# emstoudenmire/TNML

Hardware: AMD Instinct MI355X
Metric: two-site bond updates/sec (higher is better)
Workload: dtype f64; 1 GPU; fixedL N=784, maxm=120, 60000 images (BASELINE config 3: its 60 000 images on 1 GPU instead of 8), Npass=4, lambda=0.001, minm=120, fp64 throughout; random-init W at m=maxm; timed bonds 405..202 (consecutive interior bonds, Label-carrying shiftE on each, m=119); global_images=60000, sites=784, maxm=120, parallelism=dp1 (image sharding + RCCL all-reduce), rccl_ranks=1

## Files before the change

### include/tnml.h

```cpp
#ifndef TNML_H
#define TNML_H

#include <stdint.h>

#ifdef __cplusplus
extern "C" {
#endif

#define TNML_NL 10
#define TNML_MAX_PASS 64

typedef struct tnml_ctx tnml_ctx;

enum { TNML_F32 = 0, TNML_F64_E32 = 1, TNML_F64 = 2, TNML_BF16 = 3, TNML_BF16X3 = 4 };
enum { TNML_SVD_SYEVD = 0, TNML_SVD_ROCSOLVER = 1, TNML_SVD_STEDC = 2 };
enum { TNML_MODE_FIXEDL = 0, TNML_MODE_SINGLE = 1 };

typedef struct {
    int device;
    int rank, nranks;
    int N;
    int NT_local;
    int64_t NT_total;
    int maxm;
// ... 96 lines not shown
    int bond, half;
    int64_t count;
    int64_t ncorrect;
    double cost;
    double label_cost[TNML_NL];
} tnml_heldout_report;
int tnml_heldout_attach(tnml_ctx* train, tnml_ctx* heldout);
int tnml_heldout_detach(tnml_ctx* train);
int tnml_heldout_read(tnml_ctx* train, tnml_heldout_report* rep);

int tnml_truncate(const double* p, int n, int maxm, int minm, double cutoff, double* truncerr);
void tnml_sweepnext(int* b, int* ha, int N);
void tnml_shard_bounds(int64_t NT_total, int nranks, int rank, int64_t* begin, int64_t* end);

int tnml_profile_enable(tnml_ctx* ctx, int on);
int tnml_profile_select(tnml_ctx* ctx, const char* class_name);
int tnml_profile_count(tnml_ctx* ctx);
int tnml_profile_get(tnml_ctx* ctx, int idx, char* name64, int64_t* launches, double* total_ms);
int tnml_profile_reset(tnml_ctx* ctx);
int tnml_synchronize(tnml_ctx* ctx);
int tnml_set_option(tnml_ctx* ctx, const char* name, int value);
int tnml_set_option_real(tnml_ctx* ctx, const char* name, double value);
int tnml_split_stats(tnml_ctx* ctx, int64_t* spec_splits, int64_t* roll_backs, double* roll_back_ms);
int tnml_svd_stats(tnml_ctx* ctx, int64_t* fallbacks, int64_t* cluster_repairs, double* dev_before_polish, double* dev_after_first_polish);
int64_t tnml_device_bytes(tnml_ctx* ctx);

int64_t tnml_estimate_bytes(const tnml_config* cfg);
int tnml_device_memory(int device, int64_t* free_bytes, int64_t* total_bytes);
int tnml_plan_maxm(const tnml_config* cfg, int wanted, int floor_m, int64_t budget_bytes);

#define TNML_LIN_MAX_COLS 16
typedef struct tnml_lin tnml_lin;
int tnml_lin_create(tnml_lin** out, int device, int N);
int tnml_lin_destroy(tnml_lin* ctx);
const char* tnml_lin_last_error(const tnml_lin* ctx);
int tnml_lin_set_data_u8(tnml_lin* ctx, int NT, const uint8_t* pixels, const int32_t* labels);
int tnml_lin_set_data_f64(tnml_lin* ctx, int NT, const double* features, const int32_t* labels);
int tnml_lin_set_labels(tnml_lin* ctx, int K, const int32_t* labels);
int tnml_lin_cg_start(tnml_lin* ctx, const double* V, double lambda);
int tnml_lin_cg_run(tnml_lin* ctx, int npass, double* costs);
int tnml_lin_get_v(tnml_lin* ctx, double* V);
int tnml_lin_evaluate(tnml_lin* ctx, const double* V, int64_t* ncorrect, double* cnl);

#ifdef __cplusplus
}
#endif
// ... 2 lines not shown
```

### tnml_amd/csrc/kernels_res.hip

```cpp
#include "tnml_internal.h"

typedef double f64x4r __attribute__((ext_vector_type(4)));

#define FR_TI 32
#define FR_ROWS(NKA) (4 * (NKA) + 4)
#define FR_EIS(NKA) (FR_ROWS(NKA) * FR_TI)
#define FR_LDS_DOUBLES_N(NKA) (2 * FR_EIS(NKA) + 2 * 64 * FR_TI + 2 * 4 * TNML_NL * FR_TI)
#define FR_LDS_DOUBLES FR_LDS_DOUBLES_N(30)

static __device__ __forceinline__ void fr_barrier() {
    asm volatile("s_waitcnt lgkmcnt(0)" ::: "memory");
    __builtin_amdgcn_s_barrier();
    asm volatile("" ::: "memory");
}

template <int PS, int PK, int ABL, int NKA = 30, bool GEN = false, int NST = 8>
__global__ __launch_bounds__(768) void k_fwd_res(FwdResArgs A) {
    static_assert(GEN || NKA == 30, "the constant-extent form is the 120 x 120 bond");
    static_assert(NST == 8 || (NST == 4 && GEN), "four or eight streaming steps per tile");
    constexpr int EIS = FR_EIS(NKA);
    const int mI = GEN ? A.mI : 120, mO = GEN ? A.mO : 120, Kp = GEN ? A.Kp : 240, Np = GEN ? A.Np : 240;
    extern __shared__ __attribute__((aligned(16))) double fr_lds[];
    double* EIs = fr_lds;
    double* Us = EIs + 2 * EIS;
// ... 184 lines not shown
        for (int it = 1; it <= niter; ++it) {
            const long long c0 = ABL == 5 ? clock64() : 0;
            const int tile = pair + (it - 1) * npairs;
            label_dot(tile, it < niter ? tile + npairs : tile, Us + ((it - 1) & 1) * 64 * FR_TI, red + (it & 1) * 4 * TNML_NL * FR_TI, [&]() {
                x_stage(it + 1 < niter ? pair + (it + 1) * npairs : tile, (it + 1) & 1);
                if (it >= 2) finalize(pair + (it - 2) * npairs, red + ((it - 1) & 1) * 4 * TNML_NL * FR_TI);
            });
            if constexpr (NST == 8) asm volatile("s_waitcnt vmcnt(40)" ::: "memory");
            else                    asm volatile("s_waitcnt vmcnt(20)" ::: "memory");
            const long long c1 = ABL == 5 ? clock64() : 0;
            fr_barrier();
            if (ABL == 5) { const long long c2 = clock64(); t_dot += c1 - c0; t_bar += c2 - c1; }
        }
        if (ABL == 5 && A.dbg && blockIdx.x < 16 && lane == 0) { long long* d = A.dbg + (blockIdx.x * 12 + wid) * 4; d[0] = t_dot; d[1] = 0; d[2] = t_bar; d[3] = niter; }
        asm volatile("s_waitcnt vmcnt(0)" ::: "memory");
        finalize(pair + (niter - 1) * npairs, red + (niter & 1) * 4 * TNML_NL * FR_TI);
        fr_barrier();
#undef FR_WAIT
    }
}

#define SR_TI 64

template <int NKS>
__global__ __launch_bounds__(512) void k_shift_res(ShiftResArgs A) {
    constexpr int ROWS = 4 * NKS + 2;
    constexpr int NP = 2 * NKS + 1;
    extern __shared__ __attribute__((aligned(16))) double sr_lds[];
    const int tid = threadIdx.x, lane = tid & 63, w = __builtin_amdgcn_readfirstlane(tid >> 6);
    const int NTp = A.NTp, tpl = NTp / SR_TI;
    const int G = gridDim.x;
    const int niter = (A.ntiles - (int)blockIdx.x + G - 1) / G;
    const unsigned lds0 = __builtin_amdgcn_readfirstlane((unsigned)(size_t)((__attribute__((address_space(3))) char*)sr_lds));
    const unsigned doff = (unsigned)(((size_t)(lane >> 5) * NTp + 2 * (lane & 31)) * sizeof(double));
    auto dma16 = [&](const double* base, unsigned voff, unsigned dst) {
        unsigned keep;
        asm volatile("s_mov_b32 %0, m0\n\ts_mov_b32 m0, %2\n\ts_nop 0\n\tglobal_load_lds_dwordx4 %1, %3\n\ts_mov_b32 m0, %0" : "=&s"(keep) : "v"(voff), "s"(dst), "s"(base) : "memory");
    };
    const unsigned doff0 = (unsigned)((2 * (lane & 31)) * sizeof(double));
    auto stage = [&](int t, int buf) {
        const int l = t / tpl, n0 = (t - l * tpl) * SR_TI;
        const double* eb = A.EI + (size_t)l * A.EI_lstride + n0;
#pragma unroll
        for (int r = 0; r < 8; ++r) {
            int p = w + 8 * r;
            if (p >= NP) p -= NP;
            if (p >= NP) p -= NP;
            const int r0 = 2 * p < A.mI ? 2 * p : 0;
            dma16(p == NP - 1 ? A.phiI + n0 : eb + (size_t)r0 * NTp, (p != NP - 1 && 2 * p == A.mI - 1) ? doff0 : doff, lds0 + (unsigned)((buf * ROWS * SR_TI + 2 * p * SR_TI) * sizeof(double)));
        }
    };
    const int CT = A.Np >> 4;
    const bool split = CT <= 4;
    const int ct = split ? (w & 3) : w;
    const bool act = ct < CT;
    const bool do0 = !split || w < 4, do1 = !split || w >= 4;
    double me[NKS], mo[NKS];
    {
        const int g = lane >> 4, i = lane & 15;
#pragma unroll
        for (int ks = 0; ks < NKS; ++ks) {
            const bool in = act && 2 * (4 * ks + g) + 1 < A.Kp;
            me[ks] = in ? A.M[(size_t)(2 * (4 * ks + g)) * A.Np + 16 * ct + i] : 0.;
            mo[ks] = in ? A.M[(size_t)(2 * (4 * ks + g) + 1) * A.Np + 16 * ct + i] : 0.;
        }
    }
    if (niter > 0) stage(blockIdx.x, 0);
    asm volatile("s_waitcnt vmcnt(0)" ::: "memory");
    fr_barrier();
    double ob[8];
    double* obp = nullptr;
    for (int it = 0; it < niter; ++it) {
        const int t = blockIdx.x + it * G;
        const int l = t / tpl, n0 = (t - l * tpl) * SR_TI;
        int ln = lane;
        asm volatile("" : "+v"(ln));
        int g = ln >> 4, i = ln & 15;
        if (obp) {
#pragma unroll
            for (int q = 0; q < 8; ++q) { const int y = 16 * ct + g + 4 * (q & 3); if (y < A.mO) obp[(size_t)(4 * (q & 3)) * NTp + 16 * (q >> 2)] = ob[q]; }
        }
        if (it + 1 < niter) stage(t + G, (it + 1) & 1);
        const double* Eb = sr_lds + (it & 1) * ROWS * SR_TI;
        double* op = A.out + (size_t)l * A.out_lstride + (size_t)(16 * ct + g) * NTp + n0 + i;
        if (act) {
#pragma unroll
            for (int pass = 0; pass < 2; ++pass) {
                if (pass == 0 ? !do0 : !do1) continue;
                const double* ep0 = Eb + g * SR_TI + 32 * pass + i;
                const double* ep1 = ep0 + 16;
                f64x4r ce0 = {0., 0., 0., 0.}, co0 = {0., 0., 0., 0.}, ce1 = {0., 0., 0., 0.}, co1 = {0., 0., 0., 0.};
                double a0 = ep0[0], b0 = ep1[0], a1 = ep0[4 * SR_TI], b1 = ep1[4 * SR_TI];
// ... 28 lines not shown
            if (do1) obp = op + 32;
        }
        asm volatile("s_waitcnt vmcnt(0)" ::: "memory");
        fr_barrier();
    }
    if (obp) {
        const int g = lane >> 4;
#pragma unroll
        for (int q = 0; q < 8; ++q) { const int y = 16 * ct + g + 4 * (q & 3); if (y < A.mO) obp[(size_t)(4 * (q & 3)) * NTp + 16 * (q >> 2)] = ob[q]; }
    }
}

static const int sr_nks_list[] = {12, 16, 18, 20, 22, 24, 26, 28, 30};
static int sr_nks_for(int mI) {
    for (int v : sr_nks_list) if (4 * v >= mI) return v;
    return 0;
}
bool shift_res_applies(int mI, int mO) { return mI >= 33 && sr_nks_for(mI) != 0 && mO >= 1 && mO <= 128; }

template <int NKS>
static int shift_res_go(tnml_ctx* c, const ShiftResArgs& a, int grid) {
    const size_t lds = sizeof(double) * 2 * (4 * NKS + 2) * SR_TI;
    if (!c->attr_sr[NKS]) {
        if (hipFuncSetAttribute(reinterpret_cast<const void*>(k_shift_res<NKS>), hipFuncAttributeMaxDynamicSharedMemorySize, (int)lds) != hipSuccess)
            return tnml_fail(c, "shift_res: cannot reserve %zu bytes of LDS", lds);
        c->attr_sr[NKS] = true;
    }
    ProfScope ps(c, KC_FGEMM_SHIFT);
    hipLaunchKernelGGL(k_shift_res<NKS>, dim3(grid), dim3(512), lds, c->stream, a);
    return 0;
}
int launch_shift_res(tnml_ctx* c, const ShiftResArgs& a_in) {
    ShiftResArgs a = a_in;
    if (a.NTp % SR_TI) return tnml_fail(c, "shift_res: image count not a multiple of %d", SR_TI);
    if (((size_t)a.L * a.EI_lstride) * sizeof(double) >= ((size_t)1 << 32)) return tnml_fail(c, "shift_res: environment larger than 4 GB (32-bit lane offsets)");
    if (!shift_res_applies(a.mI, a.mO) || a.Np % 16 || a.Np < a.mO || a.Np > 128) return tnml_fail(c, "shift_res: bond dimensions %d x %d (packed %d) not served", a.mI, a.mO, a.Np);
    if (!c->cu_count) { hipDeviceProp_t pr; c->cu_count = hipGetDeviceProperties(&pr, c->cfg.device) == hipSuccess ? pr.multiProcessorCount : 256; }
    a.ntiles = a.L * (a.NTp / SR_TI);
    int grid = c->cu_count;
    if (c->res_grid > 0 && c->res_grid < grid) grid = c->res_grid;
    if (grid > a.ntiles) grid = a.ntiles;
    switch (sr_nks_for(a.mI)) {
        case 12: TCK((shift_res_go<12>(c, a, grid))); break;
        case 16: TCK((shift_res_go<16>(c, a, grid))); break;
        case 18: TCK((shift_res_go<18>(c, a, grid))); break;
        case 20: TCK((shift_res_go<20>(c, a, grid))); break;
        case 22: TCK((shift_res_go<22>(c, a, grid))); break;
        case 24: TCK((shift_res_go<24>(c, a, grid))); break;
        case 26: TCK((shift_res_go<26>(c, a, grid))); break;
        case 28: TCK((shift_res_go<28>(c, a, grid))); break;
        default: TCK((shift_res_go<30>(c, a, grid))); break;
    }
    HIPCK(c, hipGetLastError());
    return 0;
}

static __device__ __forceinline__ void res_wave_partials(double val, int lab, int cor, bool pap, double* out, int lane) {
    if (pap) {
        const double s = wave_sum(val);
        if (lane < 12) out[lane] = lane == 11 ? s : 0.;
        return;
    }
    double mine = 0.;
#pragma unroll
    for (int t = 0; t < TNML_NL; ++t) {
        const double s = wave_sum(lab == t ? val : 0.);
        if (lane == t) mine = s;
    }
    const double sc = wave_sum((double)cor);
    if (lane == 10) mine = sc;
    if (lane < 12) out[lane] = mine;
}

__global__ __launch_bounds__(256) void k_pfinish(PfinishArgs A) {
    const int tid = threadIdx.x, lane = tid & 63;
    const int NTp = A.NTp;
    const int ni = blockIdx.x * 256 + tid;
    if (A.conv && A.conv[0] != 0.) return;
    const int lab = A.label[ni];
// ... 106 lines not shown
```

### tnml_amd/csrc/tnml_abi.hip

```cpp
#include <algorithm>
#include <climits>
#include <cmath>
#include <cstdarg>
#include <cstdlib>
#include <cstring>

#include "tnml_internal.h"

static std::string g_create_err;

int tnml_fail(tnml_ctx* c, const char* fmt, ...) {
    char buf[512];
    va_list ap; va_start(ap, fmt); vsnprintf(buf, sizeof buf, fmt, ap); va_end(ap);
    if (c) { c->err = buf; if (c->local && c->coll_depth > 0) local_comm_abort(c); } else g_create_err = buf;
    return 1;
}
const char* tnml_last_error(const tnml_ctx* c) { return c ? c->err.c_str() : g_create_err.c_str(); }
const char* tnml_last_warning(const tnml_ctx* c) { return c ? c->warn.c_str() : ""; }
struct CollScope { tnml_ctx* c; explicit CollScope(tnml_ctx* c_) : c(c_) { ++c->coll_depth; } ~CollScope() { --c->coll_depth; } };
static int ho_locked(tnml_ctx* c, const char* who, bool train_too = false) {
    if (c->held) return tnml_fail(c, "%s: the context is attached as a held-out set (tnml_heldout_detach first)", who);
    if (train_too && c->ho) return tnml_fail(c, "%s: a held-out context is attached to this context (tnml_heldout_detach first)", who);
    return 0;
}
// ... 46 lines not shown
}
int tnml_profile_reset(tnml_ctx* c) {
    prof_resolve(c);
    for (int i = 0; i < KC_COUNT; ++i) { c->prof_launches[i] = 0; c->prof_ms[i] = 0.; }
    return 0;
}
enum OptKind { OPT_BOOL, OPT_INT, OPT_REAL };
enum OptHook { HK_NONE, HK_REUSE_P, HK_DEFER_TAIL, HK_CHECK_REPLICAS, HK_ENV_BUDGET, HK_COMM_TIMEOUT, HK_FAIL_SPLIT, HK_SVD_PRINT, HK_CG_METHOD, HK_NOISE };
struct OptDef {
    const char* name; const char* env; OptKind kind;
    int tnml_ctx::* ifield; double tnml_ctx::* rfield;
    double lo, hi; OptHook hook;
};
static const OptDef k_options[] = {
    {"fast_cg",          "TNML_FAST_CG",        OPT_BOOL, &tnml_ctx::fast_cg,             nullptr,          0, 1,       HK_NONE},
    {"reuse_p",          "TNML_REUSE_P",        OPT_BOOL, &tnml_ctx::reuse_p,             nullptr,          0, 1,       HK_REUSE_P},
    {"fuse_z",           "TNML_FUSE_Z",         OPT_BOOL, &tnml_ctx::fuse_z,              nullptr,          0, 1,       HK_NONE},
    {"merged_cg",        "TNML_MERGED_CG",      OPT_INT,  &tnml_ctx::merged_cg,           nullptr,          0, 2,       HK_NONE},
    {"defer_tail",       "TNML_DEFER_TAIL",     OPT_BOOL, &tnml_ctx::defer_tail,          nullptr,          0, 1,       HK_DEFER_TAIL},
    {"check_replicas",   "TNML_CHECK_REPLICAS", OPT_INT,  &tnml_ctx::check_replicas_mode, nullptr,          0, 2,       HK_CHECK_REPLICAS},
    {"fused_fwd",        "TNML_FUSED_FWD",      OPT_INT,  &tnml_ctx::fused_fwd,           nullptr,          0, INT_MAX, HK_NONE},
    {"fwd_res",          "TNML_FWD_RES",        OPT_INT,  &tnml_ctx::fwd_res,             nullptr,          0, 3,       HK_NONE},
    {"shift_res",        "TNML_SHIFT_RES",      OPT_INT,  &tnml_ctx::shift_res,           nullptr,          0, 2,       HK_NONE},
    {"res_grid",         nullptr,               OPT_INT,  &tnml_ctx::res_grid,            nullptr,          0, INT_MAX, HK_NONE},
    {"res_pace",         "TNML_RES_PACE",       OPT_INT,  &tnml_ctx::res_pace,            nullptr,          0, 4,       HK_NONE},
    {"grad_quad",        "TNML_GRAD_QUAD",      OPT_INT,  &tnml_ctx::grad_quad,           nullptr,          0, 2,       HK_NONE},
    {"grad_pair",        "TNML_GRAD_PAIR",      OPT_BOOL, &tnml_ctx::grad_pair,           nullptr,          0, 1,       HK_NONE},
    {"bgemm_wgs",        "TNML_BGEMM_WGS",      OPT_INT,  &tnml_ctx::bgemm_wgs,           nullptr,          0, INT_MAX, HK_NONE},
    {"bgemm_per",        "TNML_BGEMM_PER",      OPT_INT,  &tnml_ctx::bgemm_per,           nullptr,          0, 1 << 20, HK_NONE},
    {"sytrd_exit",       nullptr,               OPT_BOOL, &tnml_ctx::sytrd_exit,          nullptr,          0, 1,       HK_NONE},
    {"bgs_chol",         "TNML_BGS_CHOL",       OPT_BOOL, &tnml_ctx::bgs_chol,            nullptr,          0, 1,       HK_NONE},
    {"spec_split",       "TNML_SPEC_SPLIT",     OPT_BOOL, &tnml_ctx::spec_split,          nullptr,          0, 1,       HK_NONE},
    {"debug_fail_split", nullptr,               OPT_INT,  &tnml_ctx::debug_fail_split,    nullptr,         -1, INT_MAX, HK_FAIL_SPLIT},
    {"bf16_grad",        nullptr,               OPT_BOOL, &tnml_ctx::bf16_grad,           nullptr,          0, 1,       HK_NONE},
    {"bf16_once",        nullptr,               OPT_BOOL, &tnml_ctx::bf16_once,           nullptr,          0, 1,       HK_NONE},
    {"env_async",        nullptr,               OPT_BOOL, &tnml_ctx::env_async,           nullptr,          0, 1,       HK_NONE},
    {"env_budget_mb",    nullptr,               OPT_INT,  nullptr,                        nullptr,          0, INT_MAX, HK_ENV_BUDGET},
    {"comm_timeout_s",   nullptr,               OPT_INT,  &tnml_ctx::comm_timeout_s,      nullptr,          1, INT_MAX, HK_COMM_TIMEOUT},
    {"cg_method",        nullptr,               OPT_INT,  &tnml_ctx::cg_method,           nullptr,          0, 2,       HK_CG_METHOD},
    {"debug_nudge_rank", nullptr,               OPT_INT,  &tnml_ctx::debug_nudge_rank,    nullptr,         -1, INT_MAX, HK_NONE},
    {"mc_spin_max",      nullptr,               OPT_INT,  &tnml_ctx::mc_spin_max,         nullptr,         -1, INT_MAX, HK_NONE},
    {"svd_print",        "TNML_SVD_PRINT",      OPT_INT,  &tnml_ctx::svd_print,           nullptr,         -2, INT_MAX, HK_SVD_PRINT},
    {"fg64_cfg",         "TNML_FG64_CFG",       OPT_INT,  &tnml_ctx::opt_fg64_cfg,        nullptr,          0, 2,       HK_NONE},
    {"ldot_cfg",         "TNML_LDOT_CFG",       OPT_INT,  &tnml_ctx::opt_ldot_cfg,        nullptr,          0, 2,       HK_NONE},
    {"pcut",             nullptr,               OPT_REAL, nullptr,                        &tnml_ctx::pcut,  0, HUGE_VAL, HK_NONE},
    {"noise",            nullptr,               OPT_REAL, nullptr,                        &tnml_ctx::noise, 0, HUGE_VAL, HK_NOISE},
// ... 93 lines not shown
    c->small_elems = m * NTp;
    c->big_elems = TNML_NL * m * NTp;
    c->svd_n = 2 * c->maxm;
    c->slab_bytes = (size_t)128 * Kmax * Kmax * 4 * (c->f64() ? 2 : 1);
    c->partial_cap = (int)(NTp / 64);
    c->sM_cap = std::max(40 * m * m, (size_t)TNML_NL * Kmax * ru16(c->maxm));
    c->ebt_cap = c->bf16() ? bf16e_env_elems(c->maxm, c->NTp, c->bf16() == 2) : 0;
    c->mbt_cap = c->bf16() ? bf16e_m_elems(c->maxm, c->bf16() == 2) : 0;
    c->W.resize(c->N + 2);
    c->env.resize(c->N + 2);
    c->spare_small.assign(4, nullptr);
    c->spare_big.assign(c->c0 > 0 ? 2 : 0, nullptr);
}
struct DevBuf { void** slot; size_t bytes; bool on, site; };
static std::vector<DevBuf> device_buffers(tnml_ctx* c) {
    const size_t NTp = c->NTp, m = c->maxm, n = c->svd_n, esz = c->esz(), eesz = c->eesz(), D = sizeof(double);
    std::vector<DevBuf> v;
    auto add = [&](auto& p, size_t bytes, bool on = true) { v.push_back({(void**)&p, bytes, on, false}); };
    add(c->phi, c->N * 2 * NTp * eesz); add(c->label, NTp * sizeof(int)); add(c->ones, NTp * eesz);
    add(c->U, c->big_elems * esz); add(c->P, TNML_NL * NTp * esz); add(c->dP, TNML_NL * NTp * esz); add(c->Pp, TNML_NL * NTp * esz);
    add(c->Zp, c->small_elems * esz); add(c->Mf, c->mcap * sizeof(float)); add(c->slab, c->slab_bytes);
    add(c->partials, c->partial_cap * 12 * D); add(c->partials2, c->partial_cap * 12 * D); add(c->counters, 16 * sizeof(unsigned));
    add(c->Ppart, 2 * TNML_NL * NTp * D, c->cfg.dtype == TNML_F64 && c->cfg.mode == TNML_MODE_FIXEDL && m >= 33);
    add(c->ebt, c->ebt_cap * sizeof(unsigned short), c->bf16() != 0); add(c->mbt, c->mbt_cap * sizeof(unsigned short), c->bf16() != 0);
    add(c->vB, c->mcap * D); add(c->vR, c->mcap * D); add(c->vP, c->mcap * D); add(c->arbuf, (c->mcap + TNML_TAILN) * D); add(c->locals, 32 * D);
    add(c->scal, (SC_N + 4 * TNML_MAX_PASS) * D);
    add(c->vpart, (1024 + 16) * D);
    add(c->tB, c->mcap * D); add(c->tB2, c->mcap * D);
    add(c->sM, c->sM_cap * D); add(c->sG, n * n * D); add(c->sD, n * D); add(c->sE, 2 * n * D); add(c->sF, (n * m + 2 * TNML_NL * m * m) * D);
    add(c->sInfo, 4 * sizeof(int)); add(c->fprint, 2 * sizeof(unsigned long long));
    add(c->sE2, n * D); add(c->sTau, n * D); add(c->sV, n * n * D); add(c->sC, n * n * D);
    add(c->sW, (n + 8) * D);
    add(c->sScr, std::max<size_t>(5 * n * m, TEIG_SCRATCH_DOUBLES) * D); add(c->sS, m * m * D); add(c->sCm, m * m * D); add(c->sQ1, n * m * D); add(c->sDev, 4 * D);
    add(c->mc_xbuf, eigh_mc_xbuf_bytes(), n > 240);
    for (int j = 1; j <= c->N; ++j) v.push_back({(void**)&c->W[j].a, 2 * m * m * (j == c->c0 ? TNML_NL : 1) * D, true, true});
    for (auto& p : c->spare_small) v.push_back({(void**)&p, 2 * m * m * D, true, true});
    for (auto& p : c->spare_big) v.push_back({(void**)&p, 2 * m * m * TNML_NL * D, true, true});
    return v;
}
static int dalloc(tnml_ctx* c, void** p, size_t bytes) {
    hipError_t e = hipMalloc(p, bytes);
    if (e != hipSuccess) return tnml_fail(c, "hipMalloc of %zu bytes failed: %s", bytes, hipGetErrorString(e));
    c->bytes += (int64_t)bytes;
    return 0;
}
int ctx_alloc_doubles(tnml_ctx* c, double** p, size_t n) { return dalloc(c, (void**)p, (n ? n : 1) * sizeof(double)); }
// ... 211 lines not shown
    else if (ncclCommCount(c->comm, &cnt) != ncclSuccess) return tnml_fail(c, "ncclCommCount failed");
    if (nranks_in_comm) *nranks_in_comm = cnt;
    if (cnt != c->cfg.nranks) return tnml_fail(c, "communicator has %d ranks, context was created for %d", cnt, c->cfg.nranks);
    TCK(check_W(c));
    if (c->pend_count) return tnml_fail(c, "tnml_replica_check: a bond update is in flight");
    TCK(replica_fingerprint(c, 1, c->N, c->tail + TNML_FPSLOT));
    TCK(allreduce(c, c->tail + TNML_FPSLOT, 8));
    double h[8];
    HIPCK(c, hipMemcpyAsync(h, c->tail + TNML_FPSLOT, sizeof h, hipMemcpyDeviceToHost, c->stream));
    SYNCK(c, c->stream);
    if (!fingerprint_agrees(h, c->cfg.nranks)) return tnml_fail(c, "replicas of the weight MPS differ between ranks");
    return 0;
}

static int set_labels(tnml_ctx* c, const int32_t* labels) {
    std::vector<int> lab(c->NTp, -1);
    for (int i = 0; i < c->NT; ++i) {
        if (labels[i] < 0 || labels[i] >= TNML_NL) return tnml_fail(c, "label %d of image %d out of range", labels[i], i);
        lab[i] = labels[i];
    }
    HIPCK(c, hipMemcpy(c->label, lab.data(), sizeof(int) * c->NTp, hipMemcpyHostToDevice));
    return 0;
}
int tnml_set_data_u8(tnml_ctx* c, const uint8_t* pixels, const int32_t* labels) {
    TCK(ho_locked(c, "tnml_set_data_u8", true));
    HIPCK(c, hipSetDevice(c->cfg.device));
    TCK(set_labels(c, labels));
    uint8_t* d_pix = nullptr;
    const size_t nb = (size_t)c->NT * c->N;
    HIPCK(c, hipMalloc((void**)&d_pix, nb));
    HIPCK(c, hipMemcpy(d_pix, pixels, nb, hipMemcpyHostToDevice));
    int rc = launch_features_u8(c, d_pix, c->N, c->NT, c->NTp, c->phi);
    (void)hipStreamSynchronize(c->stream);
    (void)hipFree(d_pix);
    if (rc) return rc;
    c->data_set = true; c->currb = -1; c->p_valid = false; c->sweep_start = false;
    return 0;
}
int tnml_set_data_phi(tnml_ctx* c, const double* phi, const int32_t* labels) {
    TCK(ho_locked(c, "tnml_set_data_phi", true));
    HIPCK(c, hipSetDevice(c->cfg.device));
    TCK(set_labels(c, labels));
    const size_t ne = (size_t)c->N * 2 * c->NTp;
    if (c->env64()) {
        std::vector<double> h(ne, 0.);
        for (int i = 0; i < c->NT; ++i) for (int j = 0; j < c->N; ++j) for (int s = 0; s < 2; ++s)
            h[((size_t)j * 2 + s) * c->NTp + i] = phi[((size_t)i * c->N + j) * 2 + s];
        HIPCK(c, hipMemcpy(c->phi, h.data(), sizeof(double) * ne, hipMemcpyHostToDevice));
    } else {
        std::vector<float> h(ne, 0.f);
        for (int i = 0; i < c->NT; ++i) for (int j = 0; j < c->N; ++j) for (int s = 0; s < 2; ++s)
            h[((size_t)j * 2 + s) * c->NTp + i] = (float)phi[((size_t)i * c->N + j) * 2 + s];
        HIPCK(c, hipMemcpy(c->phi, h.data(), sizeof(float) * ne, hipMemcpyHostToDevice));
    }
    c->data_set = true; c->currb = -1; c->p_valid = false; c->sweep_start = false;
    return 0;
}

int tnml_set_site(tnml_ctx* c, int j, int ml, int mr, int has_label, const double* A) {
    TCK(ho_locked(c, "tnml_set_site", true));
    if (j < 1 || j > c->N) return tnml_fail(c, "tnml_set_site: site %d out of range", j);
    if (c->single() && has_label) return tnml_fail(c, "tnml_set_site: the per-label variant has no Label index");
    if ((j == c->c0) != (has_label != 0)) return tnml_fail(c, "Label Index not on site %d", c->c0);
    if (ml < 1 || mr < 1 || ml > c->maxm || mr > c->maxm) return tnml_fail(c, "tnml_set_site: bond dimension outside 1..maxm");
    if ((j == 1 && ml != 1) || (j == c->N && mr != 1)) return tnml_fail(c, "tnml_set_site: edge sites must have outer dimension 1");
    SiteT& s = c->W[j];
    s.ml = ml; s.mr = mr; s.L = has_label ? TNML_NL : 1; s.set = true;
    HIPCK(c, hipMemcpy(s.a, A, sizeof(double) * (size_t)ml * 2 * mr * s.L, hipMemcpyHostToDevice));
    c->currb = -1; c->p_valid = false; c->sweep_start = false;
    return 0;
}
// ... 181 lines not shown
    if (Lout_p) *Lout_p = Lout;
    c->env_epoch += 1;
    PackDesc d;
    d.TO = 1; d.L = A.L; d.st = 0; d.ss = A.ml; d.sl = (long)2 * A.ml * A.mr;
    if (from_left) { d.nx = A.ml; d.sx = 1; d.ny = A.mr; d.sy = 2 * A.ml; }
    else           { d.nx = A.mr; d.sx = 2 * A.ml; d.ny = A.ml; d.sy = 1; }
    d.Kp = ru16(2 * d.nx); d.Np = ru16(d.ny);
    if ((size_t)d.L * d.Kp * d.Np > c->sM_cap || (size_t)d.L * d.Kp * d.Np > c->mcap)
        return tnml_fail(c, "shift: packed site matrix of site %d (%d x %d x %d) exceeds the workspace", cs, d.L, d.Kp, d.Np);
    if (c->f64()) {
        TCK(launch_pack(c, d, A.a, c->sM, nullptr));
        Fgemm64Args f;
        f.EI = src ? src : c->ones;
        f.EI_lstride = (Le == TNML_NL) ? (size_t)m_in * c->NTp : 0;
        f.mI = m_in; f.phiI = phi_site(c, cs);
        f.M = c->sM; f.M_lstride = (A.L == TNML_NL) ? (size_t)d.Kp * d.Np : 0; f.Kp = d.Kp; f.Np = d.Np;
        f.phiO = nullptr;
        f.out = (double*)dst; f.out_lstride = (size_t)m_out * c->NTp; f.mO = m_out;
        f.NTp = c->NTp; f.L = Lout; f.env64 = c->env64(); f.out32 = !c->env64() && !acc_out;
        if (c->shift_res && c->env64() && !acc_out && src && Le == TNML_NL && A.L == 1 && shift_res_applies(m_in, m_out) && d.Np <= 128 &&
            (c->shift_res >= 2 || c->NTp >= 7680) &&
            (size_t)TNML_NL * m_in * c->NTp * sizeof(double) < ((size_t)1 << 32)) {
            ShiftResArgs sa{(const double*)src, (size_t)m_in * c->NTp, (const double*)phi_site(c, cs), c->sM, (double*)dst, (size_t)m_out * c->NTp, m_out, c->NTp, Lout, m_in, d.Kp, d.Np};
            return launch_shift_res(c, sa);
        }
        return launch_fgemm64(c, f);
    }
    TCK(launch_pack(c, d, A.a, nullptr, c->Mf));
    FgemmArgs f;
    f.EI = src ? (const float*)src : (const float*)c->ones;
    f.EI_lstride = (Le == TNML_NL) ? (size_t)m_in * c->NTp : 0;
    f.mI = m_in; f.phiI = (const float*)phi_site(c, cs);
    f.M = c->Mf; f.M_lstride = (A.L == TNML_NL) ? (size_t)d.Kp * d.Np : 0; f.Kp = d.Kp; f.Np = d.Np;
    f.phiO = nullptr;
    f.out = (float*)dst; f.out_lstride = (size_t)m_out * c->NTp; f.mO = m_out;
    f.NTp = c->NTp; f.L = Lout;
    return launch_fgemm(c, f);
}
static int shift_site(tnml_ctx* c, int cs, int ps, bool from_left) {
    const SiteT& A = c->W[cs];
    const bool has_prev = ps >= 1 && ps <= c->N;
    if (has_prev && !c->env[ps].built()) return tnml_fail(c, "shift: environment of site %d missing", ps);
    EnvProtect keep(c, has_prev ? ps : 0, cs, c->currb > 0 ? c->currb - 1 : 0, c->currb > 0 ? c->currb + 2 : 0);
    if (has_prev) TCK(env_ensure(c, ps));
    const int m_in = from_left ? A.ml : A.mr, m_out = from_left ? A.mr : A.ml;
    const int Le = has_prev ? c->env[ps].L : 1;
// ... 927 lines not shown
```

### tnml_amd/csrc/tnml_internal.h

```cpp
#pragma once
#include <hip/hip_runtime.h>
#include <rocblas/rocblas.h>
#include <rocsolver/rocsolver.h>
#include <rccl/rccl.h>

#include <cstdint>
#include <cstdio>
#include <string>
#include <utility>
#include <vector>

#include "../../include/tnml.h"

#define TNML_NTPAD 256

enum KClass {
    KC_FGEMM_FWD = 0, KC_FGEMM_SHIFT, KC_LABELDOT, KC_ZPRIME, KC_BGEMM, KC_SLABRED, KC_PACK, KC_VEC,
    KC_SMALLGEMM, KC_SVD, KC_ALLREDUCE, KC_PUPDATE, KC_FWD_FUSED, KC_FWD_RES, KC_GRAD_QUAD, KC_COUNT
};
static const char* const kclass_names[KC_COUNT] = {
    "fgemm_fwd", "fgemm_shift", "labeldot", "zprime", "bgemm", "slab_reduce", "pack", "cg_vec",
    "small_gemm", "svd", "allreduce", "p_update", "fwd_fused", "fwd_res", "grad_quad"};

struct EnvSlot {
// ... 135 lines not shown
    int merged_cg = 1;
    int defer_tail = 1;
    int carry_slot = -1;
    long allreduce_calls = 0, bcast_calls = 0;
    double* scal = nullptr;
    double* cgtrace = nullptr;
    double* vpart = nullptr;
    int cg_pass = 0;
    int rr_slot = 0;
    double* h_scal = nullptr;
    double *tB = nullptr, *tB2 = nullptr;
    size_t mcap = 0;
    size_t sM_cap = 0;
    double *sM = nullptr, *sG = nullptr, *sD = nullptr, *sE = nullptr, *sF = nullptr;
    double *sE2 = nullptr, *sTau = nullptr, *sV = nullptr, *sC = nullptr;
    double *sW = nullptr, *sScr = nullptr, *sS = nullptr, *sCm = nullptr, *sQ1 = nullptr, *sDev = nullptr;
    void* mc_xbuf = nullptr;
    unsigned mc_epoch = 0;
    int mc_spin_max = -1;
    bool attr_sr[32] = {false}, attr_fr[4][32] = {{false}};
    int res_pace = 0;
    int fwd_res = 1;
    int shift_res = 1;
    int res_grid = 0;
    int grad_quad = 1;
    bool attr_gq = false, attr_gp = false;
    int grad_pair = 1;
    int bgemm_per = 0;
    int bgemm_wgs = 0;
    unsigned* counters = nullptr;
    double* Ppart = nullptr;
    bool attr_sytrd = false, attr_invit = false, attr_fused = false;
    int cu_count = 0;
    int spec_split = 1; bool force_safe = false; long spec_redos = 0, spec_splits = 0;
    int debug_fail_split = -1;
    long spec_splits_total = 0; double redo_ms = 0.; std::vector<std::pair<hipEvent_t, hipEvent_t>> redo_events;
    std::vector<double*> spare_small, spare_big;
    double* hrep = nullptr;
    double* hmir = nullptr;
    double* hcost = nullptr;
    int last_dn_pairs = 0;
    size_t hrep_stride = 0;
    double svd_last_dev0 = 0., svd_last_dev1 = 0.;
    long svd_fallbacks = 0, svd_cholqr = 0;
    int svd_print = -2, svd_calls = 0, svd_dumped = 0;
    std::string svd_dump;
// ... 136 lines not shown
bool fwd_res_applies(int mI, int mO);
int launch_fwd_res(tnml_ctx* c, const FwdResArgs& a);
struct PfinishArgs {
    int npart;
    const double* Ppart;
    const double* P; const double* Pp; const double* alpha;
    const double* conv;
    const int* label; int NTp;
    double* Pout; double* dP;
    int mode;
    double* partials;
    unsigned* counter;
    double* out; int only_sum;
};
int launch_pfinish(tnml_ctx* c, const PfinishArgs& a);
struct ShiftResArgs {
    const double* EI; size_t EI_lstride;
    const double* phiI;
    const double* M;
    double* out; size_t out_lstride; int mO;
    int NTp, L;
    int mI, Kp, Np;
    int ntiles = 0;
};
bool shift_res_applies(int mI, int mO);
int launch_shift_res(tnml_ctx* c, const ShiftResArgs& a);

struct PackDesc {
    int nx, ny, TO, L;
    long sx, ss, sy, st, sl;
    int Kp, Np;
};
static inline rocblas_status dgemm_strips(rocblas_handle h, rocblas_operation ta, rocblas_operation tb, int M, int N, int K,
                                          const double* A, int lda, const double* B, int ldb, double* C, int ldc, int strips) {
    const double one = 1.0, zero = 0.0;
    if (strips <= 1 || N % strips || N / strips < 16) return rocblas_dgemm(h, ta, tb, M, N, K, &one, A, lda, B, ldb, &zero, C, ldc);
    const int ns = N / strips;
    const rocblas_stride sb = tb == rocblas_operation_none ? (rocblas_stride)ns * ldb : (rocblas_stride)ns;
    return rocblas_dgemm_strided_batched(h, ta, tb, M, ns, K, &one, A, lda, 0, B, ldb, sb, &zero, C, ldc, (rocblas_stride)ns * ldc, strips);
}
int launch_pack(tnml_ctx* c, const PackDesc& d, const double* T, double* Md, float* Mf, double* zero = nullptr, int nzero = 0);
int launch_unpack(tnml_ctx* c, const PackDesc& d, const double* Md, double* T);
int launch_cvt(tnml_ctx* c, const double* src, float* dst, size_t n);
int launch_bond_form(tnml_ctx* c, const SiteT& A1, const SiteT& A2, double* B);
int launch_cg_init(tnml_ctx* c, size_t n, double lambda, double cconv0);
int launch_cg_step(tnml_ctx* c, size_t n, double lambda, int pass, bool merged = false, const double* pp_part = nullptr, int npp = 0, bool with_update = false);
int launch_cg_resid(tnml_ctx* c, size_t n, double lambda, double cconv, int pass, bool merged = false, const double* cost_part = nullptr, int ncp = 0);
int launch_cg_fast_resid0(tnml_ctx* c, size_t n, int pass);
int launch_sqnorm(tnml_ctx* c, const double* x, size_t n, double* out);
// ... 128 lines not shown
```

### tnml_amd/fixedl.py

```python
import ctypes as C

import numpy as np

from . import lib as _lib

NL = _lib.NL


class TnmlError(RuntimeError):
    pass


class TrainStates:

    def __init__(self, labels, N, maxm, pixels=None, phi=None, device=0, rank=0, nranks=1, NT_total=None, dtype="f64",
                 single_label=None, svd_backend=0):
        self._L = _lib.load()
        self._h = C.c_void_p()
        labels = np.ascontiguousarray(labels, dtype=np.int32)
        self.NT = int(labels.shape[0])
        self.N = int(N)
        self.single = single_label is not None
        self.c0 = -1 if self.single else self.N // 2
        self.nl = 1 if self.single else NL
# ... 87 lines not shown
    def collective_stats(self):
        a, b = C.c_int64(), C.c_int64()
        self._ck(self._L.tnml_collective_stats(self._h, C.byref(a), C.byref(b)))
        return a.value, b.value

    def set_option(self, name, value):
        self._ck(self._L.tnml_set_option(self._h, name.encode(), int(value)))

    def size(self):
        return self.NT

    def synchronize(self):
        self._ck(self._L.tnml_synchronize(self._h))

    def svd_stats(self):
        fb, cr, d0, d1 = C.c_int64(), C.c_int64(), C.c_double(), C.c_double()
        self._ck(self._L.tnml_svd_stats(self._h, C.byref(fb), C.byref(cr), C.byref(d0), C.byref(d1)))
        return dict(fallbacks=fb.value, cluster_repairs=cr.value, dev_before_polish=d0.value, dev_after_first_polish=d1.value)

    def split_stats(self):
        a, b, ms = C.c_int64(), C.c_int64(), C.c_double()
        self._ck(self._L.tnml_split_stats(self._h, C.byref(a), C.byref(b), C.byref(ms)))
        return dict(speculative_splits=a.value, roll_backs=b.value, roll_back_ms=ms.value)

    def device_bytes(self):
        return self._L.tnml_device_bytes(self._h)

    def estimate_bytes(self):
        return int(self._L.tnml_estimate_bytes(C.byref(self._cfg)))

    def classify(self):
        w = np.zeros((self.NT, self.nl))
        pred = np.zeros(self.NT, dtype=np.int32)
        cnt = np.zeros(10, dtype=np.int64)
        ninc = np.zeros(10, dtype=np.int64)
        self._ck(self._L.tnml_classify(self._h, _lib.dptr(w), pred.ctypes.data_as(C.POINTER(C.c_int32)),
                                       cnt.ctypes.data_as(C.POINTER(C.c_int64)), ninc.ctypes.data_as(C.POINTER(C.c_int64))))
        return w, pred, cnt, ninc

    def set_mps(self, W):
        for j, A in enumerate(W, start=1):
            A = np.asarray(A, dtype=np.float64)
            self._ck(self._L.tnml_set_site(self._h, j, A.shape[0], A.shape[2], int(A.ndim == 4), _lib.dptr(_lib.flat(A))))

    def set_site(self, j, A):
        A = np.asarray(A, dtype=np.float64)
# ... 236 lines not shown
```

### tnml_amd/lib.py

```python
import ctypes as C
import os

import numpy as np
import torch

NL = 10
MAX_PASS = 64
DTYPES = {"f32": 0, "f64_e32": 1, "f64": 2, "bf16": 3, "bf16x3": 4}
_HERE = os.path.dirname(os.path.abspath(__file__))
LIB_PATH = os.path.join(_HERE, "libtnml.so")

EXPORTS = [
    "tnml_create", "tnml_destroy", "tnml_last_error", "tnml_comm_unique_id", "tnml_comm_init",
    "tnml_set_data_u8", "tnml_set_data_phi", "tnml_set_site", "tnml_site_dims", "tnml_get_site",
    "tnml_env_init", "tnml_set_bond", "tnml_shift_env", "tnml_env_dims", "tnml_get_env",
    "tnml_bond_dims", "tnml_bond_tensor", "tnml_forward", "tnml_gradient", "tnml_quadcost",
    "tnml_cgrad", "tnml_svd_split", "tnml_bond_update", "tnml_truncate", "tnml_sweepnext",
    "tnml_shard_bounds", "tnml_profile_enable", "tnml_profile_select", "tnml_profile_count", "tnml_profile_get",
    "tnml_profile_reset", "tnml_synchronize", "tnml_device_bytes", "tnml_svd_stats", "tnml_classify", "tnml_replica_check",
    "tnml_estimate_bytes", "tnml_device_memory", "tnml_plan_maxm", "tnml_set_option", "tnml_comm_init_local", "tnml_comm_init_oneshot", "tnml_collective_mode", "tnml_bond_update_begin", "tnml_bond_update_end", "tnml_replica_repairs", "tnml_pAp", "tnml_collective_stats", "tnml_last_warning",
    "tnml_exact", "tnml_set_option_real", "tnml_pinv", "tnml_env_stats", "tnml_oneshot_export", "tnml_oneshot_connect", "tnml_oneshot_mem_kind", "tnml_split_stats", "tnml_oneshot_region_bytes",
    "tnml_lin_create", "tnml_lin_destroy", "tnml_lin_last_error", "tnml_lin_set_data_u8", "tnml_lin_set_data_f64", "tnml_lin_set_labels",
    "tnml_lin_cg_start", "tnml_lin_cg_run", "tnml_lin_get_v", "tnml_lin_evaluate",
    "tnml_heldout_attach", "tnml_heldout_detach", "tnml_heldout_read",
]


class Config(C.Structure):
    _fields_ = [("device", C.c_int), ("rank", C.c_int), ("nranks", C.c_int), ("N", C.c_int),
                ("NT_local", C.c_int), ("NT_total", C.c_int64), ("maxm", C.c_int), ("dtype", C.c_int),
                ("svd_backend", C.c_int), ("mode", C.c_int), ("target_label", C.c_int)]


class CgTrace(C.Structure):
    _fields_ = [("npass_done", C.c_int), ("converged", C.c_int), ("cost", C.c_double * MAX_PASS),
                ("rnorm", C.c_double * MAX_PASS), ("pAp", C.c_double * MAX_PASS), ("alpha", C.c_double * MAX_PASS)]


class SweepParams(C.Structure):
    _fields_ = [("maxm", C.c_int), ("minm", C.c_int), ("cutoff", C.c_double), ("npass", C.c_int),
                ("lambda_", C.c_double), ("lambda_cost", C.c_double), ("cconv", C.c_double), ("report_costs", C.c_int)]


class BondReport(C.Structure):
# ... 61 lines not shown
    L.tnml_profile_select.argtypes = [vp, C.c_char_p]
    L.tnml_profile_count.argtypes = [vp]
    L.tnml_profile_get.argtypes = [vp, C.c_int, C.c_char_p, C.POINTER(C.c_int64), dp]
    L.tnml_profile_reset.argtypes = [vp]
    L.tnml_synchronize.argtypes = [vp]
    L.tnml_svd_stats.argtypes = [vp, C.POINTER(C.c_int64), C.POINTER(C.c_int64), dp, dp]
    L.tnml_device_bytes.argtypes = [vp]
    L.tnml_classify.argtypes = [vp, dp, C.POINTER(C.c_int32), C.POINTER(C.c_int64), C.POINTER(C.c_int64)]
    L.tnml_device_bytes.restype = C.c_int64
    L.tnml_replica_check.argtypes = [vp, ip]
    L.tnml_replica_repairs.argtypes = [vp]
    L.tnml_replica_repairs.restype = C.c_int64
    L.tnml_collective_stats.argtypes = [vp, C.POINTER(C.c_int64), C.POINTER(C.c_int64)]
    L.tnml_pAp.argtypes = [vp, dp, C.c_double, dp]
    L.tnml_last_warning.argtypes = [vp]
    L.tnml_last_warning.restype = C.c_char_p
    L.tnml_comm_init_local.argtypes = [C.POINTER(vp), C.c_int]
    L.tnml_comm_init_oneshot.argtypes = [C.POINTER(vp), C.c_int]
    L.tnml_collective_mode.argtypes = [vp]
    L.tnml_oneshot_export.argtypes = [vp, C.c_char_p]
    L.tnml_oneshot_connect.argtypes = [vp, C.c_char_p]
    L.tnml_oneshot_mem_kind.argtypes = [vp]
    L.tnml_split_stats.argtypes = [vp, C.POINTER(C.c_int64), C.POINTER(C.c_int64), C.POINTER(C.c_double)]
    L.tnml_set_option.argtypes = [vp, C.c_char_p, C.c_int]
    L.tnml_estimate_bytes.argtypes = [C.POINTER(Config)]
    L.tnml_estimate_bytes.restype = C.c_int64
    L.tnml_oneshot_region_bytes.argtypes = [C.POINTER(Config)]
    L.tnml_oneshot_region_bytes.restype = C.c_int64
    L.tnml_device_memory.argtypes = [C.c_int, C.POINTER(C.c_int64), C.POINTER(C.c_int64)]
    L.tnml_plan_maxm.argtypes = [C.POINTER(Config), C.c_int, C.c_int, C.c_int64]
    L.tnml_heldout_attach.argtypes = [vp, vp]
    L.tnml_heldout_detach.argtypes = [vp]
    L.tnml_heldout_read.argtypes = [vp, C.POINTER(HeldoutReport)]
    L.tnml_lin_create.argtypes = [C.POINTER(vp), C.c_int, C.c_int]
    L.tnml_lin_destroy.argtypes = [vp]
    L.tnml_lin_last_error.restype = C.c_char_p
    L.tnml_lin_last_error.argtypes = [vp]
    L.tnml_lin_set_data_u8.argtypes = [vp, C.c_int, C.POINTER(C.c_uint8), C.POINTER(C.c_int32)]
    L.tnml_lin_set_data_f64.argtypes = [vp, C.c_int, dp, C.POINTER(C.c_int32)]
    L.tnml_lin_set_labels.argtypes = [vp, C.c_int, C.POINTER(C.c_int32)]
    L.tnml_lin_cg_start.argtypes = [vp, dp, C.c_double]
    L.tnml_lin_cg_run.argtypes = [vp, C.c_int, dp]
    L.tnml_lin_get_v.argtypes = [vp, dp]
    L.tnml_lin_evaluate.argtypes = [vp, dp, C.POINTER(C.c_int64), dp]
    _lib = L
    return L
# ... 45 lines not shown
```

Baseline: 399.5 bond updates/s.

## Skip zero second-component phi MFMAs in shift kernel via per-tile image reorder

At data load time a new kernel classifies images per site and 64-image tile by whether the second local feature component is zero. It builds a permutation that groups those images into 16-lane groups. The fixedL fp64 shift kernel gets a specialised variant that reads this order and skips the MFMA for the zero component on such groups, then scatters results back to original image positions. This is meant to cut shift MFMA work on MNIST, where many pixels are exactly zero. In exchange it adds order tables in device memory, scattered stores and more template instantiations.

```diff
diff --git a/include/tnml.h b/include/tnml.h
--- a/include/tnml.h
+++ b/include/tnml.h
@@ -142,6 +142,7 @@
 int tnml_set_option(tnml_ctx* ctx, const char* name, int value);
 int tnml_set_option_real(tnml_ctx* ctx, const char* name, double value);
 int tnml_split_stats(tnml_ctx* ctx, int64_t* spec_splits, int64_t* roll_backs, double* roll_back_ms);
+int tnml_shift_skip_stats(tnml_ctx* ctx, int site, int64_t* groups, int64_t* skipped);
 int tnml_svd_stats(tnml_ctx* ctx, int64_t* fallbacks, int64_t* cluster_repairs, double* dev_before_polish, double* dev_after_first_polish);
 int64_t tnml_device_bytes(tnml_ctx* ctx);
 
diff --git a/tnml_amd/csrc/kernels_res.hip b/tnml_amd/csrc/kernels_res.hip
--- a/tnml_amd/csrc/kernels_res.hip
+++ b/tnml_amd/csrc/kernels_res.hip
@@ -230,7 +230,57 @@
 
 #define SR_TI 64
 
-template <int NKS>
+template <int NKS, int NG, int NSK>
+static __device__ __forceinline__ void sr_groups(const double* Eb, const double (&me)[NKS], const double (&mo)[NKS], int lane, unsigned sl, double (&ob)[16]) {
+    int ln = lane;
+    asm volatile("" : "+v"(ln));
+    int g = ln >> 4;
+    const double* ep[NG];
+    f64x4r ce[NG], co[NG];
+    double x0[NG];
+#pragma unroll
+    for (int j = 0; j < NG; ++j) {
+        ep[j] = Eb + g * SR_TI + ((sl >> (8 * j)) & 63);
+        ce[j] = f64x4r{0., 0., 0., 0.}; co[j] = f64x4r{0., 0., 0., 0.};
+    }
+#pragma unroll
+    for (int j = 0; j < NG; ++j) x0[j] = ep[j][0];
+    __builtin_amdgcn_sched_group_barrier(0x100, NG, 0);
+#pragma unroll
+    for (int ks = 0; ks < NKS; ++ks) {
+        double xa[NG];
+#pragma unroll
+        for (int j = 0; j < NG; ++j) xa[j] = x0[j];
+        if (ks + 1 < NKS) {
+#pragma unroll
+            for (int j = 0; j < NG; ++j) x0[j] = ep[j][4 * (ks + 1) * SR_TI];
+            __builtin_amdgcn_sched_group_barrier(0x100, NG, 0);
+        }
+#pragma unroll
+        for (int j = 0; j < NG; ++j) {
+            ce[j] = __builtin_amdgcn_mfma_f64_16x16x4f64(me[ks], xa[j], ce[j], 0, 0, 0);
+            if (j >= NSK) co[j] = __builtin_amdgcn_mfma_f64_16x16x4f64(mo[ks], xa[j], co[j], 0, 0, 0);
+        }
+        __builtin_amdgcn_sched_group_barrier(0x008, 2 * NG - NSK, 0);
+    }
+#pragma unroll
+    for (int j = 0; j < NG; ++j) {
+        const int im = (sl >> (8 * j)) & 63;
+        const double pI0 = Eb[(4 * NKS) * SR_TI + im];
+        if (j < NSK) {
+#pragma unroll
+            for (int e = 0; e < 4; ++e) ob[4 * j + e] = pI0 * ce[j][e];
+        } else {
+            const double pI1 = Eb[(4 * NKS + 1) * SR_TI + im];
+#pragma unroll
+            for (int e = 0; e < 4; ++e) ob[4 * j + e] = fma(pI1, co[j][e], pI0 * ce[j][e]);
+        }
+    }
+    asm volatile("" ::: "memory");
+    __builtin_amdgcn_sched_barrier(0);
+}
+
+template <int NKS, bool ZS>
 __global__ __launch_bounds__(512) void k_shift_res(ShiftResArgs A) {
     constexpr int ROWS = 4 * NKS + 2;
     constexpr int NP = 2 * NKS + 1;
@@ -276,6 +326,58 @@
     if (niter > 0) stage(blockIdx.x, 0);
     asm volatile("s_waitcnt vmcnt(0)" ::: "memory");
     fr_barrier();
+    if constexpr (ZS) {
+        auto slots = [&](int t, int ln) {
+            const uint8_t* o = A.ord + (size_t)(t % tpl) * SR_TI + (ln & 15);
+            return (unsigned)o[0] | (unsigned)o[16] << 8 | (unsigned)o[32] << 16 | (unsigned)o[48] << 24;
+        };
+        auto put = [&](int t, int ln, unsigned psl, const double (&ob)[16]) {
+            const int l = t / tpl, n0 = (t - l * tpl) * SR_TI, g = ln >> 4;
+            double* op = A.out + (size_t)l * A.out_lstride + (size_t)(16 * ct + g) * NTp + n0;
+#pragma unroll
+            for (int q = 0; q < 16; ++q) {
+                const int y = 16 * ct + g + 4 * (q & 3);
+                if (y < A.mO && (q < 8 || !split)) op[(size_t)(4 * (q & 3)) * NTp + ((psl >> (8 * (q >> 2))) & 63)] = ob[q];
+            }
+        };
+        unsigned sl = 0, sln = 0, psl = 0;
+        if (niter > 0) sl = slots(blockIdx.x, lane);
+        double ob[16];
+        for (int it = 0; it < niter; ++it) {
+            const int t = blockIdx.x + it * G;
+            int ln = lane;
+            asm volatile("" : "+v"(ln));
+            if (act && it > 0) put(t - G, ln, psl, ob);
+            if (it + 1 < niter) { stage(t + G, (it + 1) & 1); sln = slots(t + G, ln); }
+            const double* Eb = sr_lds + (it & 1) * ROWS * SR_TI;
+            if (act) {
+                const int s = __builtin_amdgcn_readfirstlane((int)(((sl >> 6) & 3) | ((sl >> 12) & 4)));
+                if (!split) {
+                    switch (s) {
+                        case 0:  sr_groups<NKS, 4, 0>(Eb, me, mo, lane, sl, ob); break;
+                        case 1:  sr_groups<NKS, 4, 1>(Eb, me, mo, lane, sl, ob); break;
+                        case 2:  sr_groups<NKS, 4, 2>(Eb, me, mo, lane, sl, ob); break;
+                        case 3:  sr_groups<NKS, 4, 3>(Eb, me, mo, lane, sl, ob); break;
+                        default: sr_groups<NKS, 4, 4>(Eb, me, mo, lane, sl, ob); break;
+                    }
+                    psl = sl;
+                } else {
+                    const int s2 = w < 4 ? (s < 2 ? s : 2) : (s > 2 ? s - 2 : 0);
+                    psl = w < 4 ? sl : sl >> 16;
+                    switch (s2) {
+                        case 0:  sr_groups<NKS, 2, 0>(Eb, me, mo, lane, psl, ob); break;
+                        case 1:  sr_groups<NKS, 2, 1>(Eb, me, mo, lane, psl, ob); break;
+                        default: sr_groups<NKS, 2, 2>(Eb, me, mo, lane, psl, ob); break;
+                    }
+                }
+            }
+            asm volatile("s_waitcnt vmcnt(0)" : "+v"(sln) :: "memory");
+            sl = sln;
+            fr_barrier();
+        }
+        if (act && niter > 0) put(blockIdx.x + (niter - 1) * G, lane, psl, ob);
+        return;
+    }
     double ob[8];
     double* obp = nullptr;
     for (int it = 0; it < niter; ++it) {
@@ -350,12 +452,14 @@
 static int shift_res_go(tnml_ctx* c, const ShiftResArgs& a, int grid) {
     const size_t lds = sizeof(double) * 2 * (4 * NKS + 2) * SR_TI;
     if (!c->attr_sr[NKS]) {
-        if (hipFuncSetAttribute(reinterpret_cast<const void*>(k_shift_res<NKS>), hipFuncAttributeMaxDynamicSharedMemorySize, (int)lds) != hipSuccess)
+        if (hipFuncSetAttribute(reinterpret_cast<const void*>(k_shift_res<NKS, false>), hipFuncAttributeMaxDynamicSharedMemorySize, (int)lds) != hipSuccess ||
+            hipFuncSetAttribute(reinterpret_cast<const void*>(k_shift_res<NKS, true>), hipFuncAttributeMaxDynamicSharedMemorySize, (int)lds) != hipSuccess)
             return tnml_fail(c, "shift_res: cannot reserve %zu bytes of LDS", lds);
         c->attr_sr[NKS] = true;
     }
     ProfScope ps(c, KC_FGEMM_SHIFT);
-    hipLaunchKernelGGL(k_shift_res<NKS>, dim3(grid), dim3(512), lds, c->stream, a);
+    if (a.ord && a.nz) hipLaunchKernelGGL((k_shift_res<NKS, true>), dim3(grid), dim3(512), lds, c->stream, a);
+    else               hipLaunchKernelGGL((k_shift_res<NKS, false>), dim3(grid), dim3(512), lds, c->stream, a);
     return 0;
 }
 int launch_shift_res(tnml_ctx* c, const ShiftResArgs& a_in) {
@@ -383,6 +487,29 @@
     return 0;
 }
 
+__global__ __launch_bounds__(256) void k_shift_order(const double* __restrict__ phi, int N, int NTp, uint8_t* __restrict__ ord, uint8_t* __restrict__ nz, int* __restrict__ cnt) {
+    const int lane = threadIdx.x & 63, tpl = NTp / SR_TI;
+    const size_t wave = (size_t)blockIdx.x * 4 + (threadIdx.x >> 6);
+    if (wave >= (size_t)N * tpl) return;
+    const int j = (int)(wave / tpl), ti = (int)(wave - (size_t)j * tpl);
+    const bool z = phi[((size_t)j * 2 + 1) * NTp + (size_t)ti * SR_TI + lane] == 0.0;
+    const unsigned long long mz = __ballot(z), below = ((unsigned long long)1 << lane) - 1;
+    const int nzc = __popcll(mz);
+    const int slot = z ? __popcll(mz & below) : nzc + __popcll(~mz & below);
+    const int sk = nzc >> 4, code = slot < 16 ? (sk & 3) : (slot < 32 ? sk >> 2 : 0);
+    ord[((size_t)j * tpl + ti) * SR_TI + slot] = (uint8_t)(lane | code << 6);
+    if (lane == 0) { nz[(size_t)j * tpl + ti] = (uint8_t)nzc; if (nzc >= 16) atomicAdd(cnt + j, nzc >> 4); }
+}
+int launch_shift_order(tnml_ctx* c, const double* phi, int N, int NTp, uint8_t* ord, uint8_t* nz, int* cnt) {
+    if (NTp % SR_TI) return tnml_fail(c, "shift_order: image count not a multiple of %d", SR_TI);
+    ProfScope ps(c, KC_PACK);
+    HIPCK(c, hipMemsetAsync(cnt, 0, sizeof(int) * N, c->stream));
+    const size_t waves = (size_t)N * (NTp / SR_TI);
+    hipLaunchKernelGGL(k_shift_order, dim3((unsigned)((waves + 3) / 4)), dim3(256), 0, c->stream, phi, N, NTp, ord, nz, cnt);
+    HIPCK(c, hipGetLastError());
+    return 0;
+}
+
 static __device__ __forceinline__ void res_wave_partials(double val, int lab, int cor, bool pap, double* out, int lane) {
     if (pap) {
         const double s = wave_sum(val);
diff --git a/tnml_amd/csrc/tnml_abi.hip b/tnml_amd/csrc/tnml_abi.hip
--- a/tnml_amd/csrc/tnml_abi.hip
+++ b/tnml_amd/csrc/tnml_abi.hip
@@ -92,6 +92,7 @@
     {"fused_fwd",        "TNML_FUSED_FWD",      OPT_INT,  &tnml_ctx::fused_fwd,           nullptr,          0, INT_MAX, HK_NONE},
     {"fwd_res",          "TNML_FWD_RES",        OPT_INT,  &tnml_ctx::fwd_res,             nullptr,          0, 3,       HK_NONE},
     {"shift_res",        "TNML_SHIFT_RES",      OPT_INT,  &tnml_ctx::shift_res,           nullptr,          0, 2,       HK_NONE},
+    {"shift_skip",       "TNML_SHIFT_SKIP",     OPT_BOOL, &tnml_ctx::shift_skip,          nullptr,          0, 1,       HK_NONE},
     {"res_grid",         nullptr,               OPT_INT,  &tnml_ctx::res_grid,            nullptr,          0, INT_MAX, HK_NONE},
     {"res_pace",         "TNML_RES_PACE",       OPT_INT,  &tnml_ctx::res_pace,            nullptr,          0, 4,       HK_NONE},
     {"grad_quad",        "TNML_GRAD_QUAD",      OPT_INT,  &tnml_ctx::grad_quad,           nullptr,          0, 2,       HK_NONE},
@@ -231,6 +232,8 @@
     add(c->Zp, c->small_elems * esz); add(c->Mf, c->mcap * sizeof(float)); add(c->slab, c->slab_bytes);
     add(c->partials, c->partial_cap * 12 * D); add(c->partials2, c->partial_cap * 12 * D); add(c->counters, 16 * sizeof(unsigned));
     add(c->Ppart, 2 * TNML_NL * NTp * D, c->cfg.dtype == TNML_F64 && c->cfg.mode == TNML_MODE_FIXEDL && m >= 33);
+    const bool zs = c->cfg.dtype == TNML_F64 && c->cfg.mode == TNML_MODE_FIXEDL && m >= 33;
+    add(c->zs_ord, c->N * NTp, zs); add(c->zs_nz, c->N * (NTp / 64), zs); add(c->zs_cnt, c->N * sizeof(int), zs);
     add(c->ebt, c->ebt_cap * sizeof(unsigned short), c->bf16() != 0); add(c->mbt, c->mbt_cap * sizeof(unsigned short), c->bf16() != 0);
     add(c->vB, c->mcap * D); add(c->vR, c->mcap * D); add(c->vP, c->mcap * D); add(c->arbuf, (c->mcap + TNML_TAILN) * D); add(c->locals, 32 * D);
     add(c->scal, (SC_N + 4 * TNML_MAX_PASS) * D);
@@ -488,6 +491,22 @@
     HIPCK(c, hipMemcpy(c->label, lab.data(), sizeof(int) * c->NTp, hipMemcpyHostToDevice));
     return 0;
 }
+static int shift_order_build(tnml_ctx* c) {
+    if (!c->zs_ord) return 0;
+    TCK(launch_shift_order(c, (const double*)c->phi, c->N, c->NTp, c->zs_ord, c->zs_nz, c->zs_cnt));
+    c->zs_groups.assign(c->N, 0);
+    HIPCK(c, hipMemcpyAsync(c->zs_groups.data(), c->zs_cnt, sizeof(int) * c->N, hipMemcpyDeviceToHost, c->stream));
+    SYNCK(c, c->stream);
+    return 0;
+}
+int tnml_shift_skip_stats(tnml_ctx* c, int site, int64_t* groups, int64_t* skipped) {
+    if (!c) return tnml_fail(c, "tnml_shift_skip_stats: null argument");
+    if (site < 1 || site > c->N) return tnml_fail(c, "tnml_shift_skip_stats: site %d out of range", site);
+    if (!c->zs_ord || !c->data_set || c->zs_groups.size() != (size_t)c->N) return tnml_fail(c, "tnml_shift_skip_stats: this context has no tile order tables (fp64 storage, fixedL, maxm >= 33, data set)");
+    if (groups) *groups = (int64_t)(c->NTp / 16);
+    if (skipped) *skipped = c->zs_groups[site - 1];
+    return 0;
+}
 int tnml_set_data_u8(tnml_ctx* c, const uint8_t* pixels, const int32_t* labels) {
     TCK(ho_locked(c, "tnml_set_data_u8", true));
     HIPCK(c, hipSetDevice(c->cfg.device));
@@ -500,6 +519,7 @@
     (void)hipStreamSynchronize(c->stream);
     (void)hipFree(d_pix);
     if (rc) return rc;
+    TCK(shift_order_build(c));
     c->data_set = true; c->currb = -1; c->p_valid = false; c->sweep_start = false;
     return 0;
 }
@@ -513,6 +533,7 @@
         for (int i = 0; i < c->NT; ++i) for (int j = 0; j < c->N; ++j) for (int s = 0; s < 2; ++s)
             h[((size_t)j * 2 + s) * c->NTp + i] = phi[((size_t)i * c->N + j) * 2 + s];
         HIPCK(c, hipMemcpy(c->phi, h.data(), sizeof(double) * ne, hipMemcpyHostToDevice));
+        TCK(shift_order_build(c));
     } else {
         std::vector<float> h(ne, 0.f);
         for (int i = 0; i < c->NT; ++i) for (int j = 0; j < c->N; ++j) for (int s = 0; s < 2; ++s)
@@ -740,6 +761,7 @@
             (c->shift_res >= 2 || c->NTp >= 7680) &&
             (size_t)TNML_NL * m_in * c->NTp * sizeof(double) < ((size_t)1 << 32)) {
             ShiftResArgs sa{(const double*)src, (size_t)m_in * c->NTp, (const double*)phi_site(c, cs), c->sM, (double*)dst, (size_t)m_out * c->NTp, m_out, c->NTp, Lout, m_in, d.Kp, d.Np};
+            if (c->shift_skip && c->zs_ord) { sa.ord = c->zs_ord + (size_t)(cs - 1) * c->NTp; sa.nz = c->zs_nz + (size_t)(cs - 1) * (c->NTp / 64); }
             return launch_shift_res(c, sa);
         }
         return launch_fgemm64(c, f);
diff --git a/tnml_amd/csrc/tnml_internal.h b/tnml_amd/csrc/tnml_internal.h
--- a/tnml_amd/csrc/tnml_internal.h
+++ b/tnml_amd/csrc/tnml_internal.h
@@ -181,6 +181,9 @@
     int res_pace = 0;
     int fwd_res = 1;
     int shift_res = 1;
+    int shift_skip = 1;
+    uint8_t* zs_ord = nullptr; uint8_t* zs_nz = nullptr; int* zs_cnt = nullptr;
+    std::vector<int> zs_groups;
     int res_grid = 0;
     int grad_quad = 1;
     bool attr_gq = false, attr_gp = false;
@@ -363,9 +366,12 @@
     int NTp, L;
     int mI, Kp, Np;
     int ntiles = 0;
+    const uint8_t* ord = nullptr;
+    const uint8_t* nz = nullptr;
 };
 bool shift_res_applies(int mI, int mO);
 int launch_shift_res(tnml_ctx* c, const ShiftResArgs& a);
+int launch_shift_order(tnml_ctx* c, const double* phi, int N, int NTp, uint8_t* ord, uint8_t* nz, int* cnt);
 
 struct PackDesc {
     int nx, ny, TO, L;
diff --git a/tnml_amd/fixedl.py b/tnml_amd/fixedl.py
--- a/tnml_amd/fixedl.py
+++ b/tnml_amd/fixedl.py
@@ -133,6 +133,11 @@
         a, b, ms = C.c_int64(), C.c_int64(), C.c_double()
         self._ck(self._L.tnml_split_stats(self._h, C.byref(a), C.byref(b), C.byref(ms)))
         return dict(speculative_splits=a.value, roll_backs=b.value, roll_back_ms=ms.value)
+
+    def shift_skip_stats(self, j):
+        a, b = C.c_int64(), C.c_int64()
+        self._ck(self._L.tnml_shift_skip_stats(self._h, int(j), C.byref(a), C.byref(b)))
+        return a.value, b.value
 
     def device_bytes(self):
         return self._L.tnml_device_bytes(self._h)
diff --git a/tnml_amd/lib.py b/tnml_amd/lib.py
--- a/tnml_amd/lib.py
+++ b/tnml_amd/lib.py
@@ -19,7 +19,7 @@
     "tnml_shard_bounds", "tnml_profile_enable", "tnml_profile_select", "tnml_profile_count", "tnml_profile_get",
     "tnml_profile_reset", "tnml_synchronize", "tnml_device_bytes", "tnml_svd_stats", "tnml_classify", "tnml_replica_check",
     "tnml_estimate_bytes", "tnml_device_memory", "tnml_plan_maxm", "tnml_set_option", "tnml_comm_init_local", "tnml_comm_init_oneshot", "tnml_collective_mode", "tnml_bond_update_begin", "tnml_bond_update_end", "tnml_replica_repairs", "tnml_pAp", "tnml_collective_stats", "tnml_last_warning",
-    "tnml_exact", "tnml_set_option_real", "tnml_pinv", "tnml_env_stats", "tnml_oneshot_export", "tnml_oneshot_connect", "tnml_oneshot_mem_kind", "tnml_split_stats", "tnml_oneshot_region_bytes",
+    "tnml_exact", "tnml_set_option_real", "tnml_pinv", "tnml_env_stats", "tnml_oneshot_export", "tnml_oneshot_connect", "tnml_oneshot_mem_kind", "tnml_split_stats", "tnml_oneshot_region_bytes", "tnml_shift_skip_stats",
     "tnml_lin_create", "tnml_lin_destroy", "tnml_lin_last_error", "tnml_lin_set_data_u8", "tnml_lin_set_data_f64", "tnml_lin_set_labels",
     "tnml_lin_cg_start", "tnml_lin_cg_run", "tnml_lin_get_v", "tnml_lin_evaluate",
     "tnml_heldout_attach", "tnml_heldout_detach", "tnml_heldout_read",
@@ -127,6 +127,7 @@
     L.tnml_oneshot_connect.argtypes = [vp, C.c_char_p]
     L.tnml_oneshot_mem_kind.argtypes = [vp]
     L.tnml_split_stats.argtypes = [vp, C.POINTER(C.c_int64), C.POINTER(C.c_int64), C.POINTER(C.c_double)]
+    L.tnml_shift_skip_stats.argtypes = [vp, C.c_int, C.POINTER(C.c_int64), C.POINTER(C.c_int64)]
     L.tnml_set_option.argtypes = [vp, C.c_char_p, C.c_int]
     L.tnml_estimate_bytes.argtypes = [C.POINTER(Config)]
     L.tnml_estimate_bytes.restype = C.c_int64
```

Measured after the change: 406.0 bond updates/s (median of 6 runs). +1.6%, better.
